# febrianrachmadi/dep-gan-im

Hardware: AMD Instinct MI355X
Metric: 2D slices/sec (G+2D+GP train step), 256x256x1 fp32 (higher is better)
Workload: dtype f32; 1 GPU; DEP-GAN-IM twoCritics canonical train step (critic-Y2 + critic-DEM + G update, WGAN-GP), batch 32 per GPU, 256x256x1; per_gpu_batch=32, global_batch=32, parallelism=dp1

## Files before the change

### dep_gan_im_amd/csrc/igemm_wino.hip

```cpp
#include <stdlib.h>

#include <type_traits>

#include "common.h"
#include "epilogue.h"

namespace {

constexpr int WN_CK = 8;
constexpr int WN_TW = 18;
constexpr int WN_CP = 36;
constexpr int WN_XV = WN_CK / 4;

template <int MT>
struct WnCfg {
  static constexpr int TH = 8 * MT;
  static constexpr int NTILE = 32 * MT;
  static constexpr int PIXT = (TH + 2) * WN_TW;
  static constexpr int XTOT = PIXT * WN_XV;
  static constexpr int NXP = (XTOT + 255) / 256;
  static constexpr int RAW = NXP * 256 * 4;
  static constexpr int VPLANE = NTILE * WN_CK;
  static constexpr int V = 16 * VPLANE;
  static constexpr int ZPLANE = NTILE * WN_CP + 32;
  static constexpr int Z = 8 * ZPLANE;
  static constexpr size_t LDS = sizeof(float) * (size_t)((2 * RAW + V) > Z ? (2 * RAW + V) : Z);
  static constexpr int WGS_PER_CU = (MT == 2) ? 2 : 3;
};

static __device__ __forceinline__ int rslot(int pix, int half) { return (2 * pix + half) ^ (((pix >> 2) & 1) << 1); }

static __device__ __forceinline__ int vslot(int T, int cg, int a) { return ((2 * T + cg) ^ ((T >> 2) & 1) ^ (a << 1)) << 2; }

template <int MT, bool PERS, bool HEAD, int ABL = 0>
static __device__ __forceinline__ void wino_body(const ConvArgs& a) {
  typedef WnCfg<MT> C;
  constexpr int MF = 32, NT = 32;
  constexpr int WN_RAW = C::RAW, WN_VPLANE = C::VPLANE, WN_ZPLANE = C::ZPLANE, WN_XTOT = C::XTOT, NXP = C::NXP;
  typedef f32x16 acc_t;
  extern __shared__ __attribute__((aligned(16))) float smem[];
  float* const raw0 = smem;
  float* const raw1 = smem + WN_RAW;
  float* V = smem + 2 * WN_RAW;

  const int tid = threadIdx.x;
  const int lane = tid & 63, wv = tid >> 6;
  const int r = lane & 31, h = lane >> 5;
  const int tilesX = (a.W + 15) >> 4, tilesY = (a.H + C::TH - 1) / C::TH;
  const unsigned nNTall = (unsigned)a.lgy, nPix = (unsigned)a.lgx;
  const int nCC = a.Cin / WN_CK;

  constexpr int SENT = (int)0x80000000;
  int xvo[NXP], xyx[NXP];
#pragma unroll
  for (int i = 0; i < NXP; ++i) {
    const int q = tid + i * 256;
    const int lq = q ^ (((q >> 3) & 1) << 1);
    const int pix = lq >> 1, part = lq & 1;
    const int ly = pix / WN_TW, lx = pix - ly * WN_TW;
    xvo[i] = (q < WN_XTOT) ? 4 * (ly * (int)a.in.sY + lx * (int)a.in.sX + part * 4) : SENT;
    xyx[i] = (ly << 8) | lx;
  }
  int tA[MT][4], tB[MT][4], tV[MT];
  float tS[MT];
#pragma unroll
  for (int i = 0; i < MT; ++i) {
    const int q = lane + 64 * i;
    const int cg = q & 1, aa = wv, T = q >> 1;
    const int tyi = T >> 3, txi = T & 7;
    const int rA = (aa == 0) ? 0 : (aa == 2 ? 2 : 1), rB = (aa == 3) ? 3 : (aa == 2 ? 1 : 2);
#pragma unroll
    for (int j = 0; j < 4; ++j) {
      tA[i][j] = 4 * rslot((2 * tyi + rA) * WN_TW + 2 * txi + j, cg);
      tB[i][j] = 4 * rslot((2 * tyi + rB) * WN_TW + 2 * txi + j, cg);
    }
    tV[i] = (4 * aa) * WN_VPLANE + vslot(T, cg, aa);
    tS[i] = (aa == 1) ? 1.f : -1.f;
  }
  const int wbase = __builtin_amdgcn_readfirstlane(wv * 256);
  int aoff[MT];
#pragma unroll
  for (int mt = 0; mt < MT; ++mt) aoff[mt] = vslot(32 * mt + r, h, wv);
  const int boff = (4 * wv * 32 + r) * WN_CK + 4 * h;

  unsigned id = blockIdx.x;
  do {
    int t, ntile;
    if ((nPix & 7u) == 0) {
      const unsigned x = id & 7u, sl = id >> 3;
      ntile = (int)(sl % nNTall);
      t = (int)(x * (nPix >> 3) + sl / nNTall);
    } else {
      t = (int)(id % nPix);
      ntile = (int)(id / nPix);
    }
    const int tx0 = (t % tilesX) * 16;
    t /= tilesX;
    const int ty0 = (t % tilesY) * C::TH;
    const int b = t / tilesY;
    const long out_goff = 0;
    const int n0 = ntile * NT;
    const float* inb = a.in.p + (long)b * a.in.sB;
    const bool interior = ty0 >= 1 && ty0 + C::TH + 1 <= a.H && tx0 >= 1 && tx0 + 17 <= a.W;
    const char* halo0 = reinterpret_cast<const char*>(inb + ((long)(ty0 - 1) * a.in.sY + (long)(tx0 - 1) * a.in.sX));
    auto coff = [&](int cc) -> long {
      if (a.cpt > 0) {
        const int run = cc / a.cpt;
        return a.in_run_off[run] + (long)(cc - run * a.cpt) * WN_CK;
      }
      return (long)cc * WN_CK;
    };
    const float* const xorg = a.in.p - ((long)a.in.sY + (long)a.in.sX);
    const unsigned long long xu = (unsigned long long)xorg;
    const unsigned xlo = __builtin_amdgcn_readfirstlane((unsigned)xu), xhi = __builtin_amdgcn_readfirstlane((unsigned)(xu >> 32));
    const __amdgpu_buffer_rsrc_t rx =
        __builtin_amdgcn_make_buffer_rsrc((void*)(((unsigned long long)xhi << 32) | xlo), 0, 0x7FFFFFFF, 0x00020000);
    const int xso0 = 4 * (b * (int)a.in.sB + ty0 * (int)a.in.sY + tx0 * (int)a.in.sX);
    auto stage_dma = [&](int cc, int buf) {
      const int xso = xso0 + 4 * (int)coff(cc);
      float* xs = (buf ? raw1 : raw0) + wbase;
      if (interior) {
#pragma unroll
        for (int i = 0; i < NXP; ++i) {
          const int vo = xvo[i];
          __builtin_amdgcn_raw_ptr_buffer_load_lds(rx, (__attribute__((address_space(3))) void*)(xs + i * 1024), 16, vo,
                                                   xso, 0, 0);
        }
      } else {
#pragma unroll
        for (int i = 0; i < NXP; ++i) {
          const int iy = ty0 + (xyx[i] >> 8) - 1, ix = tx0 + (xyx[i] & 255) - 1;
          const int vo = (iy >= 0 && iy < a.H && ix >= 0 && ix < a.W) ? xvo[i] : SENT;
          __builtin_amdgcn_raw_ptr_buffer_load_lds(rx, (__attribute__((address_space(3))) void*)(xs + i * 1024), 16, vo,
                                                   xso, 0, 0);
        }
      }
    };

    acc_t acc[4][MT];

    const float* wnt = a.w + (size_t)ntile * nCC * (16 * NT * WN_CK) + boff;
    if (!(ABL & 8)) stage_dma(0, 0);
    auto chunk = [&](const int cc, auto first_tag) {
      constexpr bool FIRST = decltype(first_tag)::value;
      f32x4 bq[4];
#pragma unroll
      for (int f = 0; f < 4; ++f)
        bq[f] = *reinterpret_cast<const f32x4*>(wnt + (size_t)cc * (16 * NT * WN_CK) + f * (NT * WN_CK));
      asm volatile("s_waitcnt vmcnt(0)" ::: "memory");
      __syncthreads();
      if (!(ABL & 8) && cc + 1 < nCC) stage_dma(cc + 1, (cc + 1) & 1);
      const float* raw = (cc & 1) ? raw1 : raw0;
#pragma unroll
      for (int i = 0; i < ((ABL & 2) ? 0 : MT); ++i) {
        f32x4 tc[4];
#pragma unroll
        for (int j = 0; j < 4; ++j) {
          const f32x4 x = *reinterpret_cast<const f32x4*>(raw + tA[i][j]);
          const f32x4 y = *reinterpret_cast<const f32x4*>(raw + tB[i][j]);
#pragma unroll
          for (int k = 0; k < 4; ++k) tc[j][k] = fmaf(y[k], tS[i], x[k]);
        }
        f32x4 v0, v1, v2, v3;
#pragma unroll
        for (int k = 0; k < 4; ++k) {
          v0[k] = tc[0][k] - tc[2][k];
          v1[k] = tc[1][k] + tc[2][k];
          v2[k] = tc[2][k] - tc[1][k];
          v3[k] = tc[1][k] - tc[3][k];
        }
        *reinterpret_cast<f32x4*>(V + tV[i]) = v0;
        *reinterpret_cast<f32x4*>(V + tV[i] + WN_VPLANE) = v1;
        *reinterpret_cast<f32x4*>(V + tV[i] + 2 * WN_VPLANE) = v2;
        *reinterpret_cast<f32x4*>(V + tV[i] + 3 * WN_VPLANE) = v3;
      }
      f32x4 av[2][MT];
      auto load_a = [&](int f, f32x4* d) {
#pragma unroll
        for (int mt = 0; mt < MT; ++mt)
          d[mt] = *reinterpret_cast<const f32x4*>(V + (4 * wv + f) * WN_VPLANE + aoff[mt]);
      };
      load_a(0, av[0]);
#pragma unroll
      for (int f = 0; f < 4; ++f) {
        if (f + 1 < 4) load_a(f + 1, av[(f + 1) & 1]);
        __builtin_amdgcn_sched_barrier(0);
#pragma unroll
        for (int j = 0; j < 4; ++j)
#pragma unroll
          for (int mt = 0; mt < MT; ++mt)
            if (!(ABL & 4)) {
              if (FIRST && j == 0) {
                const acc_t zero = {0.f, 0.f, 0.f, 0.f, 0.f, 0.f, 0.f, 0.f, 0.f, 0.f, 0.f, 0.f, 0.f, 0.f, 0.f, 0.f};
                acc[f][mt] = __builtin_amdgcn_mfma_f32_32x32x2f32(bq[f][j], av[f & 1][mt][j], zero, 0, 0, 0);
              } else {
                acc[f][mt] = __builtin_amdgcn_mfma_f32_32x32x2f32(bq[f][j], av[f & 1][mt][j], acc[f][mt], 0, 0, 0);
              }
            } else {
              if (FIRST && j == 0) acc[f][mt] = acc_t{};
              acc[f][mt][j] += bq[f][j] * av[f & 1][mt][j];
            }
        __builtin_amdgcn_sched_barrier(0);
      }
    };
    chunk(0, std::true_type{});
    for (int cc = 1; cc < nCC; ++cc) chunk(cc, std::false_type{});

    if (ABL & 1) {
      float sacc = 0.f;
#pragma unroll
      for (int f = 0; f < 4; ++f)
#pragma unroll
        for (int mt = 0; mt < MT; ++mt)
#pragma unroll
          for (int j = 0; j < 16; ++j) sacc += acc[f][mt][j];
      if (sacc == 12345.678f) a.out.p[tid] = sacc;
      __syncthreads();
      continue;
    }
    auto zstage = [&]() {
      __syncthreads();
      float* zw = smem + (2 * wv) * WN_ZPLANE + r * WN_CP + 4 * h;
#pragma unroll
      for (int mt = 0; mt < MT; ++mt)
#pragma unroll
        for (int g = 0; g < 4; ++g) {
          f32x4 z0, z1;
#pragma unroll
          for (int k = 0; k < 4; ++k) {
            const float m0 = acc[0][mt][4 * g + k], m1 = acc[1][mt][4 * g + k], m2 = acc[2][mt][4 * g + k],
                        m3 = acc[3][mt][4 * g + k];
            z0[k] = (m0 + m1) + m2;
            z1[k] = (m1 - m2) - m3;
          }
          *reinterpret_cast<f32x4*>(zw + mt * (32 * WN_CP) + 8 * g) = z0;
          *reinterpret_cast<f32x4*>(zw + WN_ZPLANE + mt * (32 * WN_CP) + 8 * g) = z1;
        }
      __syncthreads();
    };
#define EPI_PRE_SYNC
#define EPI_STAGE
#define EPI_STAGE_LATE zstage()
#define EPI_NPASS (4 * MT)
#define EPI_OYW (ty0 + 2 * MT * __builtin_amdgcn_readfirstlane(wv))
#define EPI_FULL ((ty0 + C::TH <= a.H) && (tx0 + 16 <= a.W))
#define EPI_FETCH(v, py, px)                                                                                         \
  {                                                                                                                  \
    const float* zb = smem + ((px)&1) * WN_ZPLANE +                                                                  \
                      ((MT * __builtin_amdgcn_readfirstlane(wv) + ((py) >> 1)) * 8 + ((px) >> 1)) * WN_CP + c4;       \
    const f32x4 za = *reinterpret_cast<const f32x4*>(zb + (((py)&1) ? 2 : 0) * WN_ZPLANE);                           \
    const f32x4 zb1 = *reinterpret_cast<const f32x4*>(zb + (((py)&1) ? 4 : 2) * WN_ZPLANE);                          \
    const f32x4 zc = *reinterpret_cast<const f32x4*>(zb + (((py)&1) ? 6 : 4) * WN_ZPLANE);                           \
    _Pragma("unroll") for (int k_ = 0; k_ < 4; ++k_) v[k_] = ((py)&1) ? (za[k_] - zb1[k_]) - zc[k_] : (za[k_] + zb1[k_]) + zc[k_]; \
  }
#define EPI_HEAD HEAD
#include "igemm_epilogue.inc"
#undef EPI_HEAD
#undef EPI_FETCH
#undef EPI_FULL
#undef EPI_OYW
#undef EPI_NPASS
#undef EPI_STAGE_LATE
#undef EPI_STAGE
#undef EPI_PRE_SYNC
    if (PERS) __syncthreads();
  } while (PERS && (id += gridDim.x) < nPix * nNTall);
}

template <int MT, bool PERS>
__global__ __launch_bounds__(256, WnCfg<MT>::WGS_PER_CU) void wino_conv_kernel(const ConvArgs a) {
  wino_body<MT, PERS, false>(a);
}
template <bool PERS>
__global__ __launch_bounds__(256, 2) void wino_conv_head_kernel(const ConvArgs a) {
  wino_body<2, PERS, true>(a);
}
#ifdef DEPGAN_WINO_ABLATIONS
template <int MT, int ABL>
__global__ __launch_bounds__(256, WnCfg<MT>::WGS_PER_CU) void wino_conv_abl_kernel(const ConvArgs a) {
  wino_body<MT, true, false, ABL>(a);
}
#endif

}

bool dg_conv_wino_supported(const ConvPlan& pl, const ConvArgs& a) {
  if (!dg_plan_wino(pl)) return false;
  if (a.Cin != pl.Cin || (a.Cin % WN_CK) || (a.Cout % 32) || a.groups > 1 || a.dbg || ((a.H | a.W) & 1)) return false;
  if (a.cpt > 0 && ((a.Cin % (a.cpt * WN_CK)) != 0 || a.Cin / (a.cpt * WN_CK) > 4)) return false;
  return true;
}

static int wino_mt(const ConvArgs& a) {
  static int forced = -1;
  if (forced < 0) {
    const char* e = getenv("DEPGAN_WINO_MT");
    forced = e ? atoi(e) : 0;
  }
  if (a.ep.head_out) return 2;
  if (forced == 1 || forced == 2) return forced;
  return 1;
}

template <int MT>
static void wino_geometry(ConvArgs& a, long* total, long* G, bool* pers) {
  a.lgx = cdiv(a.W, 16) * cdiv(a.H, WnCfg<MT>::TH) * a.B;
  a.lgy = a.Cout / 32;
  *total = (long)a.lgx * a.lgy;
  const long cap = (long)WnCfg<MT>::WGS_PER_CU * dg_cu_count();
  *pers = *total > cap;
  *G = *pers ? cap : *total;
}

const char* dg_conv_wino_name(const ConvArgs& a_in) {
  ConvArgs a = a_in;
  long total, G;
  bool pers;
  const int mt = wino_mt(a);
  if (mt == 2) wino_geometry<2>(a, &total, &G, &pers); else wino_geometry<1>(a, &total, &G, &pers);
  if (a.ep.head_out) return pers ? "wino_conv_head_kernel<true>" : "wino_conv_head_kernel<false>";
  if (mt == 2) return pers ? "wino_conv_kernel<2,true>" : "wino_conv_kernel<2,false>";
  return pers ? "wino_conv_kernel<1,true>" : "wino_conv_kernel<1,false>";
}

template <int MT>
static int wino_launch(ConvArgs a, hipStream_t st) {
  long total, G;
  bool pers;
  wino_geometry<MT>(a, &total, &G, &pers);
  constexpr size_t LDS = WnCfg<MT>::LDS;
  static DgOncePerDevice once;
  if (once.need()) {
    HIPCHECK(hipFuncSetAttribute(reinterpret_cast<const void*>(&wino_conv_kernel<MT, false>),
                                 hipFuncAttributeMaxDynamicSharedMemorySize, (int)LDS));
    HIPCHECK(hipFuncSetAttribute(reinterpret_cast<const void*>(&wino_conv_kernel<MT, true>),
                                 hipFuncAttributeMaxDynamicSharedMemorySize, (int)LDS));
    if (MT == 2) {
      HIPCHECK(hipFuncSetAttribute(reinterpret_cast<const void*>(&wino_conv_head_kernel<false>),
                                   hipFuncAttributeMaxDynamicSharedMemorySize, (int)LDS));
      HIPCHECK(hipFuncSetAttribute(reinterpret_cast<const void*>(&wino_conv_head_kernel<true>),
                                   hipFuncAttributeMaxDynamicSharedMemorySize, (int)LDS));
    }
  }
#ifdef DEPGAN_WINO_ABLATIONS
  if (const char* e = getenv("DEPGAN_WINO_ABL")) {
    const int abl = atoi(e);
    if (abl && pers && !a.ep.head_out) {
#define WN_ABL_CASE(N)                                                                                              \
  case N:                                                                                                           \
    HIPCHECK(hipFuncSetAttribute(reinterpret_cast<const void*>(&wino_conv_abl_kernel<MT, N>),                       \
                                 hipFuncAttributeMaxDynamicSharedMemorySize, (int)LDS));                            \
    hipLaunchKernelGGL((wino_conv_abl_kernel<MT, N>), dim3((unsigned)G), dim3(256), LDS, st, a);                    \
    break;
// ... 32 lines not shown
```

### dep_gan_im_amd/csrc/op_entries.hip

```cpp
#include "model.h"
#include "train_ops.h"

#include <math.h>
#include <stdlib.h>
#include <stdio.h>
#include <string.h>

int op_pack_jobs(PackJob* jobs, int n, hipStream_t st) {
  const unsigned nb = dg_pack_layout(jobs, n);
  DevTmp jd(st);
  DGCHECK(jd.alloc(n * sizeof(PackJob)));
  hipError_t e = hipMemcpyAsync(jd.p, jobs, n * sizeof(PackJob), hipMemcpyHostToDevice, st);
  if (e != hipSuccess) { dg_set_error("op_pack_jobs: upload failed: %s", hipGetErrorString(e)); return DG_ERR_HIP; }
  return dg_pack_weights_batch(jd.as<PackJob>(), n, nb, st);
}

extern "C" {

static int op_conv_run(ConvArgs a, const float* w_hwio, int Cin, int Cout, int KS, int path, int bwd, hipStream_t st) {
  const int ci = a.Cin, co = a.Cout;
  ConvPlan pl = (path == 3) ? dg_plan_conv_bf16(KS, ci, co)
                : (path == 4 || path == 5) ? dg_plan_conv_split(KS, ci, co, path == 5 ? 3 : 2)
                : (path == 6) ? dg_plan_conv_items(KS, ci, co, 1L << 30) : dg_plan_conv(KS, ci, co);
  if (path == 7) pl = dg_plan_conv_items(KS, ci, co, 1L << 30);
// ... 60 lines not shown
}

int depgan_op_conv2d(const float* in, const float* w_hwio, const float* bias, float* out, int B, int H, int W,
                     int Cin, int Cout, int KS, int relu, int path, void* stream) {
  return op_conv(in, w_hwio, bias, out, B, H, W, Cin, Cout, KS, relu, path, 0, (hipStream_t)stream);
}
int depgan_op_conv2d_bwd_data(const float* dy, const float* w_hwio, float* dx, int B, int H, int W, int Cin,
                              int Cout, int KS, int path, void* stream) {
  return op_conv(dy, w_hwio, nullptr, dx, B, H, W, Cin, Cout, KS, 0, path, 1, (hipStream_t)stream);
}
int depgan_op_conv2d_wgrad(const float* x, const float* dy, float* dw, int B, int H, int W, int Cin, int Cout, int KS,
                           void* stream) {
  hipStream_t st = (hipStream_t)stream;
  const bool big = (Cin % 4 == 0 && Cout % 4 == 0 && Cin >= 8);
  const size_t pf = big ? dg_wgrad_part_floats(KS, B, H, W, Cin, Cout) : dg_wgrad_small_part_floats(KS, B, H, W, Cin, Cout);
  DevTmp part(st);
  DGCHECK(part.alloc(pf * sizeof(float)));
  WgradArgs a = wgrad_args(make_view(const_cast<float*>(x), H, W, Cin), make_view(const_cast<float*>(dy), H, W, Cout),
                           part.as<float>(), B, H, W, Cin, Cout);
  int nch = 0;
  DGCHECK(big ? dg_wgrad(KS, a, &nch, st) : dg_wgrad_small(KS, a, &nch, st));
  return dg_wgrad_reduce(a.part, nch, KS * KS, Cin, Cout, nullptr, dw, nullptr, 0, 0, st);
}
int depgan_op_conv2d_wgrad_bf16(const float* x, const float* dy, float* dw, int B, int H, int W, int Cin, int Cout,
                                int KS, void* stream) {
  hipStream_t st = (hipStream_t)stream;
  if (!dg_wgrad_bf16_supported(KS, Cin, Cout)) { dg_set_error("op_wgrad_bf16: shape not covered"); return DG_ERR_UNSUPPORTED; }
  const size_t pf = dg_wgrad_bf16_part_floats(KS, B, H, W, Cin, Cout);
  DevTmp part(st);
  DGCHECK(part.alloc(pf * sizeof(float)));
  WgradArgs a = wgrad_args(make_view(const_cast<float*>(x), H, W, Cin), make_view(const_cast<float*>(dy), H, W, Cout),
                           part.as<float>(), B, H, W, Cin, Cout);
  int nch = 0;
  DGCHECK(dg_wgrad_bf16(KS, a, &nch, st));
  return dg_wgrad_reduce(a.part, nch, KS * KS, Cin, Cout, nullptr, dw, nullptr, 0, 0, st);
}
int depgan_op_deconv2x2(const float* in, const float* w_hwoi, const float* bias, const float* scale,
                        const float* shift, float* out, int B, int H, int W, int Cin, int Cout, int relu,
                        void* stream) {
  if (!in || !w_hwoi || !out || B < 1 || H < 1 || W < 1) { dg_set_error("op_deconv2x2: bad argument"); return DG_ERR_ARG; }
  DeconvArgs d;
  memset(&d, 0, sizeof(d));
  d.in = in;
  d.w = w_hwoi;
  d.out = make_view(out, 2 * H, 2 * W, Cout);
  d.bias = bias; d.scale = scale; d.shift = shift; d.relu = relu;
  d.H = H; d.W = W; d.Cin = Cin; d.Cout = Cout;
  return dg_deconv_fwd(d, B, (hipStream_t)stream);
}
int depgan_op_deconv2x2_wgrad(const float* in, const float* dout, float* dw_hwoi, float* colsum, int B, int H, int W,
                              int Cin, int Cout, void* stream) {
  if (!in || !dout || !dw_hwoi || B < 1 || H < 1 || W < 1) { dg_set_error("op_deconv2x2_wgrad: bad argument"); return DG_ERR_ARG; }
  hipStream_t st = (hipStream_t)stream;
  DeconvWgradArgs d;
  memset(&d, 0, sizeof(d));
  d.in = in;
  d.dout = make_view(const_cast<float*>(dout), 2 * H, 2 * W, Cout);
  d.H = H; d.W = W; d.Cin = Cin; d.Cout = Cout;
  if (!dg_deconv_wgrad_supported(B, H, W, Cin, Cout, make_view(const_cast<float*>(in), H, W, Cin), d.dout)) {
    dg_set_error("op_deconv2x2_wgrad: shape %dx%dx%d %d->%d not covered by the fused kernel", B, H, W, Cin, Cout);
    return DG_ERR_UNSUPPORTED;
  }
  const size_t pf = dg_deconv_wgrad_part_floats(B, H, W, Cin, Cout);
  DevTmp part(st), col(st);
  DGCHECK(part.alloc(pf * sizeof(float)));
  if (col.alloc((pf / ((size_t)Cin * Cout)) * Cout * sizeof(float)) != DG_OK) {
    dg_set_error("op_deconv2x2_wgrad: out of memory");
    return DG_ERR_HIP;
  }
  d.part = part.as<float>();
  d.colpart = colsum ? col.as<float>() : nullptr;
  int nch = 0;
  DGCHECK(dg_deconv_wgrad(d, B, &nch, st));
  return dg_wgrad_finish_rows(d.part, nch, 4, Cin, Cout, nullptr, dw_hwoi, nullptr, 0, 1, d.colpart, 4 * nch, Cout, nullptr,
                              colsum, nullptr, st);
}
int depgan_op_maxpool(const float* in, float* out, int B, int Ho, int Wo, int C, void* stream) {
  return dg_maxpool(make_view(const_cast<float*>(in), 2 * Ho, 2 * Wo, C), make_view(out, Ho, Wo, C), B, Ho, Wo, C,
                    (hipStream_t)stream);
}

int depgan_eval_accumulate(const float* pred, const float* mask, double* acc, long n, void* stream) {
  if (!pred || !acc || n < 0) { dg_set_error("eval_accumulate: null argument"); return DG_ERR_ARG; }
  return dg_eval_accumulate(pred, mask, acc, (size_t)n, (hipStream_t)stream);
}
int depgan_eval_divide(double* acc, long n, double divisor, void* stream) {
  if (!acc || n < 0) { dg_set_error("eval_divide: null argument"); return DG_ERR_ARG; }
  return dg_eval_divide(acc, (size_t)n, divisor, (hipStream_t)stream);
}
int depgan_eval_counts(const float* x, int nicg, const double* pred, const float* code_real, const float* mask1,
                       const float* wmh1, const float* mask2, const float* wmh2, const float* prob2, long npix,
                       double thr, long long out_host[DEPGAN_EVAL_NCOUNT], void* stream) {
  if (!x || !pred || !out_host || nicg < 1 || npix < 0) { dg_set_error("eval_counts: bad argument"); return DG_ERR_ARG; }
  hipStream_t st = (hipStream_t)stream;
  DevTmp dev(st);
  DGCHECK(dev.alloc(DEPGAN_EVAL_NCOUNT * sizeof(unsigned long long)));
  DGCHECK(dg_eval_counts(x, nicg, pred, code_real, mask1, wmh1, mask2, wmh2, prob2, (size_t)npix, thr,
                         dev.as<unsigned long long>(), st));
  unsigned long long h[DEPGAN_EVAL_NCOUNT];
  if (hipMemcpyAsync(h, dev.p, sizeof(h), hipMemcpyDeviceToHost, st) != hipSuccess ||
      hipStreamSynchronize(st) != hipSuccess) {
    dg_set_error("eval_counts: copy back failed");
    return DG_ERR_HIP;
  }
  for (int k = 0; k < DEPGAN_EVAL_NCOUNT; ++k) out_host[k] = (long long)h[k];
  return DG_OK;
}


static int op_alloc(DevTmp* t, size_t floats, const char* who) {
  if (t->alloc((floats ? floats : 1) * sizeof(float)) != DG_OK) {
    dg_set_error("%s: out of device memory (%zu floats)", who, floats);
    return DG_ERR_HIP;
  }
  return DG_OK;
}
static size_t op_scratch(long scratch_floats, size_t need) { return scratch_floats > 0 ? (size_t)scratch_floats : need; }


int depgan_op_conv2d_fused(const float* in, long isB, long isY, long isX, const float* w_hwio, const float* bias,
                           const float* scale, const float* shift, const float* film_mul, const float* film_add,
                           int film_ld, float* out, long osB, long osY, long osX, float* out_pre, long psB, long psY,
                           long psX, const float* res, long rsB, long rsY, long rsX, const float* mask, long msB,
                           long msY, long msX, float* pool, long qsB, long qsY, long qsX, const float* head_w,
                           const float* head_b, float* head_out, int head_tanh, int head_skip_out, int B, int H, int W,
                           int Cin, int Cout, int KS, int relu, int accumulate, int path, int bwd, void* stream) {
  if (op_view_bad_batched(in, isB, isY, isX) || op_view_bad_batched(out, osB, osY, osX) || !w_hwio || B < 1 || H < 1 || W < 1 || Cin < 1 ||
      Cout < 1 || (KS != 1 && KS != 3 && KS != 5) || (out_pre && op_view_bad_batched(out_pre, psB, psY, psX)) ||
      (res && op_view_bad_batched(res, rsB, rsY, rsX)) || (mask && op_view_bad_batched(mask, msB, msY, msX)) ||
      (pool && op_view_bad_batched(pool, qsB, qsY, qsX))) {
    dg_set_error("op_conv2d_fused: null or non-positive argument");
    return DG_ERR_ARG;
  }
  const int co = bwd ? Cin : Cout;
  if (!scale != !shift || !film_mul != !film_add || (film_mul && film_ld < co)) {
    dg_set_error("op_conv2d_fused: scale / shift and film_mul / film_add come in pairs, film_ld >= output channels");
    return DG_ERR_ARG;
  }
  if ((head_w || head_b || head_out) && !(head_w && head_b && head_out)) { dg_set_error("op_conv2d_fused: null head argument"); return DG_ERR_ARG; }
  if (head_skip_out && !head_out) { dg_set_error("op_conv2d_fused: head_skip_out without a head"); return DG_ERR_ARG; }
  if (path < 1 || path > 10) { dg_set_error("op_conv2d_fused: path must be 1 ... 10"); return DG_ERR_ARG; }
  ConvArgs a = conv_args(op_view(in, isB, isY, isX), op_view(out, osB, osY, osX), B, H, W, bwd ? Cout : Cin, co);
  Epilogue& e = a.ep;
  e.bias = bias; e.scale = scale; e.shift = shift;
  e.film_mul = film_mul; e.film_add = film_add; e.film_ld = film_ld;
  e.out_pre = op_view_or_null(out_pre, psB, psY, psX);
  e.res = op_view_or_null(res, rsB, rsY, rsX);
  e.mask = op_view_or_null(mask, msB, msY, msX);
  e.pool = op_view_or_null(pool, qsB, qsY, qsX);
  e.relu = relu; e.accumulate = accumulate;
  e.head_w = head_w; e.head_b = head_b; e.head_out = head_out;
  e.head_tanh = head_tanh; e.head_skip_out = head_skip_out;
  return op_conv_run(a, w_hwio, Cin, Cout, KS, path, bwd ? 1 : 0, (hipStream_t)stream);
}


int depgan_op_deconv2x2_igemm(int form, const float* in, long isB, long isY, long isX, const float* w_hwoi,
                              const float* bias, const float* scale, const float* shift, float* out, long osB, long osY,
                              long osX, const float* mask, long msB, long msY, long msX, int B, int H, int W, int Cin,
                              int Cout, int relu, int path, void* stream) {
  if (op_view_bad_batched(in, isB, isY, isX) || op_view_bad_batched(out, osB, osY, osX) || !w_hwoi || B < 1 || H < 1 || W < 1 || Cin < 1 ||
      Cout < 1 || (mask && op_view_bad_batched(mask, msB, msY, msX))) {
    dg_set_error("op_deconv2x2_igemm: null or non-positive argument");
    return DG_ERR_ARG;
  }
  if (form < 0 || form > 2 || !scale != !shift || (path != 1 && path != 3 && path != 8)) {
    dg_set_error("op_deconv2x2_igemm: form must be 0, 1 or 2, path 1, 3 or 8, scale and shift come as a pair");
    return DG_ERR_ARG;
  }
  if (form == 0 ? mask != nullptr : (bias || scale || relu)) {
    dg_set_error("op_deconv2x2_igemm: the forward takes bias / scale / shift / relu, the backward-data forms a mask");
    return DG_ERR_ARG;
  }
  if (path == 8) { dg_set_error("op_deconv2x2_igemm: the Winograd kernel has no 1x1 form"); return DG_ERR_UNSUPPORTED; }
  auto plan = [&](int ci, int co) { return path == 3 ? dg_plan_conv_bf16(1, ci, co) : dg_plan_conv(1, ci, co); };
  auto covered = [&](const ConvPlan& p) { return dg_plan_mfma(p) && (path == 3) == dg_plan_bf16(p); };
  hipStream_t st = (hipStream_t)stream;
  ConvArgs a = conv_args(null_view(), null_view(), B, H, W, 0, 0);
  DevTmp wt(st);
  if (form == 0) {
    const ConvPlan pf = plan(Cin, Cout);
    if (!covered(pf)) { dg_set_error("op_deconv2x2_igemm: no MFMA plan for %d -> %d on path %d", Cin, Cout, path); return DG_ERR_UNSUPPORTED; }
    const TView o = op_view(out, osB, osY, osX);
    a.in = op_view(in, isB, isY, isX);
    a.Cin = Cin; a.Cout = Cout;
    a.ep.bias = bias; a.ep.scale = scale; a.ep.shift = shift; a.ep.relu = relu;
    DGCHECK(wt.alloc(4 * pf.packedFloats * sizeof(float)));
    const float* panels[4];
    for (int t = 0; t < 4; ++t) {
      float* dst = wt.as<float>() + (size_t)t * pf.packedFloats;
      DGCHECK(dg_pack_weights(pf, w_hwoi + (size_t)t * Cout * Cin, Cin, Cout, 1, 0, 0, nullptr, dst, st));
      panels[t] = dst;
    }
    deconv_groups(&a, o, panels);
    return dg_conv_igemm(pf, a, st);
  }
  const ConvPlan pb = plan(Cout, Cin);
  if (!covered(pb)) { dg_set_error("op_deconv2x2_igemm: no MFMA plan for %d -> %d on path %d", Cout, Cin, path); return DG_ERR_UNSUPPORTED; }
  const TView d = op_view(in, isB, isY, isX);
  a.out = op_view(out, osB, osY, osX);
  a.Cout = Cin;
  a.ep.mask = op_view_or_null(mask, msB, msY, msX);
  if (form == 1) {
    const ConvPlan pbf = plan(4 * Cout, Cin);
    if (!(pbf.family == pb.family && pbf.planes == pb.planes && (Cout % pb.CK) == 0 && pbf.packedFloats == 4 * pb.packedFloats)) {
      dg_set_error("op_deconv2x2_igemm: the gathered 1x1 form does not cover %d -> %d", Cout, Cin);
      return DG_ERR_UNSUPPORTED;
    }
    DGCHECK(wt.alloc(pbf.packedFloats * sizeof(float)));
    const size_t blk = (size_t)pb.nCC * pb.NT * pb.CK;
    PackJob jobs[4];
    for (int t = 0; t < 4; ++t) {
      float* dst = reinterpret_cast<float*>(wt.as<char>() + t * blk * dg_plan_elem_bytes(pb));
      DGCHECK(dg_pack_job(pb, w_hwoi + (size_t)t * Cout * Cin, Cin, Cout, 1, 1, 0, nullptr, dst, 4 * blk, &jobs[t]));
    }
    DGCHECK(op_pack_jobs(jobs, 4, st));
    deconv_gather_k(&a, d, Cout, pb.CK);
    a.w = wt.as<float>();
    return dg_conv_igemm(pbf, a, st);
  }
  DGCHECK(wt.alloc(4 * pb.packedFloats * sizeof(float)));
  a.Cin = Cout;
  for (int t = 0; t < 4; ++t) {
    float* dst = wt.as<float>() + (size_t)t * pb.packedFloats;
    DGCHECK(dg_pack_weights(pb, w_hwoi + (size_t)t * Cout * Cin, Cin, Cout, 1, 1, 0, nullptr, dst, st));
    a.in = strided2(d, t / 2, t % 2);
    a.w = dst;
    a.ep.accumulate = (t > 0);
    DGCHECK(dg_conv_igemm(pb, a, st));
  }
  return DG_OK;
}

int depgan_op_conv2d_wgrad_ex(const float* x, long xsB, long xsY, long xsX, const float* dy, long dsB, long dsY,
                              long dsX, const float* scale, float* dw, float* raw, int accumulate, int oi,
                              int colB, const float* colscale, float* colout, float* colraw, int B, int H, int W,
                              int Cin, int Cout, int KS, int bf16, void* stream) {
  if (op_view_bad_batched(x, xsB, xsY, xsX) || op_view_bad_batched(dy, dsB, dsY, dsX) || !dw || B < 1 || H < 1 || W < 1 || Cin < 1 || Cout < 1 ||
      (KS != 1 && KS != 3 && KS != 5)) {
    dg_set_error("op_conv2d_wgrad_ex: null or non-positive argument");
    return DG_ERR_ARG;
  }
  const bool cols = colout || colraw;
  if ((bf16 != 0 && bf16 != 1) || (cols ? (colB < 1 || colB > B) : (colB != 0 || colscale != nullptr))) {
    dg_set_error("op_conv2d_wgrad_ex: bf16 must be 0 or 1; column sums need colout or colraw and 1 <= colB <= B");
    return DG_ERR_ARG;
  }
  const bool mfma = Cin % 4 == 0 && Cout % 4 == 0 && Cin >= 8;
  if (bf16 && !(mfma && dg_wgrad_bf16_supported(KS, Cin, Cout))) {
    dg_set_error("op_conv2d_wgrad_ex: the bf16 weight-gradient kernel does not cover %d -> %d", Cin, Cout);
    return DG_ERR_UNSUPPORTED;
  }
  hipStream_t st = (hipStream_t)stream;
  WgradWs ws;
  memset(&ws, 0, sizeof(ws));
  ws.partFloats = bf16 ? dg_wgrad_bf16_part_floats(KS, B, H, W, Cin, Cout)
                  : mfma ? dg_wgrad_part_floats(KS, B, H, W, Cin, Cout) : dg_wgrad_small_part_floats(KS, B, H, W, Cin, Cout);
  ws.scratchFloats = mfma ? ws.partFloats / ((size_t)KS * KS * Cin) : (cols ? dg_colsum_scratch(colB, H, W, Cout) : 0);
  ws.bf16 = bf16 != 0;
  ws.st = st;
  DevTmp part(st), scratch(st);
  DGCHECK(op_alloc(&part, ws.partFloats, "op_conv2d_wgrad_ex"));
  DGCHECK(op_alloc(&scratch, ws.scratchFloats, "op_conv2d_wgrad_ex"));
  ws.part = part.as<float>();
  ws.scratch = scratch.as<float>();
  const ColSum cs = {colB, colscale, colout, colraw};
  return wgrad_run(ws, KS, op_view(x, xsB, xsY, xsX), op_view(dy, dsB, dsY, dsX), B, H, W, Cin, Cout, scale, dw, raw, accumulate,
                   oi, cols ? &cs : nullptr);
}

int depgan_debug_wgrad_plan(int kernel, int KS, int B, int H, int W, int Cin, int Cout, int out[4]) {
  if (!out || B < 1 || H < 1 || W < 1 || Cin < 1 || Cout < 1) {
    dg_set_error("debug_wgrad_plan: null or non-positive argument");
    return DG_ERR_ARG;
  }
  switch (kernel) {
    case 0: return dg_wgrad_plan(KS, B, H, W, Cin, Cout, out);
    case 1: return dg_wgrad_small_plan(KS, B, H, W, Cin, Cout, out);
    case 2: return dg_wgrad_bf16_plan(KS, B, H, W, Cin, Cout, out);
    case 3: return dg_wgrad_bf16s_plan(KS, B, H, W, Cin, Cout, out);
    case 4: return dg_deconv_wgrad_plan(B, H, W, Cin, Cout, out);
  }
  dg_set_error("debug_wgrad_plan: kernel %d is not one of 0..4", kernel);
  return DG_ERR_ARG;
}


int depgan_op_bn_moments(const float* x, long sB, long sY, long sX, int B, int H, int W, int C, float* mean, float* var,
                         long scratch_floats, void* stream) {
  if (!x || !mean || !var || B < 1 || H < 1 || W < 1 || C < 4) { dg_set_error("op_bn_moments: bad argument"); return DG_ERR_ARG; }
  hipStream_t st = (hipStream_t)stream;
  const size_t cap = op_scratch(scratch_floats, dg_col_moments_scratch(B, H, W, C));
  DevTmp scratch(st);
  DGCHECK(op_alloc(&scratch, cap, "op_bn_moments"));
  return dg_col_moments(op_view(x, sB, sY, sX), B, H, W, C, mean, var, scratch.as<float>(), cap, st);
}

int depgan_op_bn_backward(const float* dy, const float* raw, float* draw, long sB, long sY, long sX, int B, int H, int W,
                          int C, const float* gamma, const float* mean, const float* var, float eps, float invN,
                          float dyscale, float* dgamma, float* dbeta, long scratch_floats, void* stream) {
  if (!dy || !raw || !draw || !gamma || !mean || !var || !dgamma || !dbeta || B < 1 || H < 1 || W < 1 || C < 4) {
    dg_set_error("op_bn_backward: bad argument");
    return DG_ERR_ARG;
  }
  hipStream_t st = (hipStream_t)stream;
  const size_t cap = op_scratch(scratch_floats, dg_colsum_pair_scratch(B, H, W, C));
// ... 334 lines not shown
```

### include/depgan.h

```cpp
#ifndef DEPGAN_H
#define DEPGAN_H
#include <stddef.h>
#ifdef __cplusplus
extern "C" {
#endif

typedef struct depgan_ctx depgan_ctx;

#define DEPGAN_ABI_VERSION 3
int depgan_abi_version(void);
size_t depgan_config_size(void);
const char* depgan_source_hash(void);

typedef struct depgan_config {
  int struct_size;
  int batch;
  int height;
  int width;
  int nicg;
  int first_fm;
  float im_thresh;
  float delta;
  float lrD, lrG;
  float beta1, beta2, adam_eps;
// ... 30 lines not shown
float* depgan_arena_ptr(depgan_ctx* ctx, int net, int arena);
int depgan_weights_changed(depgan_ctx* ctx, int net);

int depgan_g_forward(depgan_ctx* ctx, const float* x_dev, const float* z_dev, float* out_dev, int n);
int depgan_d_forward(depgan_ctx* ctx, int net, const float* img_dev, float* out_dev, int n);

int depgan_critic_grads(depgan_ctx* ctx, int net, const float* y2_dev, const float* x_dev, const float* z_dev,
                        const float* ep_dev, float out_host[2]);
int depgan_critic_step(depgan_ctx* ctx, int net, const float* y2_dev, const float* x_dev, const float* z_dev,
                       const float* ep_dev, float out_host[2]);
int depgan_g_eval(depgan_ctx* ctx, const float* x_dev, const float* y2_dev, const float* z_dev, float out_host[6]);
int depgan_g_grads(depgan_ctx* ctx, const float* x_dev, const float* y2_dev, const float* z_dev, float out_host[6]);
#define DEPGAN_MAX_MULTI 32
int depgan_g_eval_multi(depgan_ctx* ctx, const float* x_dev, const float* y2_dev, const float* z_all_dev, int k,
                        float* out_host, float* sums_host);
int depgan_g_step(depgan_ctx* ctx, const float* x_dev, const float* y2_dev, const float* z_dev, float out_host[6]);
int depgan_apply_adam(depgan_ctx* ctx, int net);
long depgan_get_adam_step(depgan_ctx* ctx, int net);
int depgan_set_adam_step(depgan_ctx* ctx, int net, long t);

#define DEPGAN_MAX_CRITIC_STEPS 256
int depgan_gen_iteration(depgan_ctx* ctx, const float* x_y2, const float* y2_y2, const float* z_y2, const float* ep_y2,
                         int n_y2, const float* x_dem, const float* y2_dem, const float* z_dem, const float* ep_dem,
                         int n_dem, long batch_stride, const float* x_gen, const float* y2_gen, const float* z_gen, int k,
                         float* out_host, int* best_host);

int depgan_uresnet_grads(depgan_ctx* ctx, const float* x_dev, const float* z_dev, const float* labels_dev, int n,
                         unsigned drop_seed, float* loss_host);
int depgan_uresnet_step(depgan_ctx* ctx, const float* x_dev, const float* z_dev, const float* labels_dev, int n,
                        unsigned drop_seed, float* loss_host);
int depgan_uresnet_eval(depgan_ctx* ctx, const float* x_dev, const float* z_dev, const float* labels_dev, int n,
                        float* loss_host);

int depgan_last_sums(depgan_ctx* ctx, float out_host[8]);

int depgan_profile_enable(depgan_ctx* ctx, int on);
int depgan_profile_read(depgan_ctx* ctx, int klass, double* total_ms, long* launches, double* flops);
int depgan_profile_read_bytes(depgan_ctx* ctx, int klass, double* bytes);
int depgan_profile_reset(depgan_ctx* ctx);
int depgan_profile_dump(depgan_ctx* ctx, const char* path);

#define DEPGAN_EVAL_NCOUNT 20
int depgan_eval_accumulate(const float* pred_dev, const float* mask_dev, double* acc_dev, long n, void* stream);
int depgan_eval_divide(double* acc_dev, long n, double divisor, void* stream);
int depgan_eval_counts(const float* x_dev, int nicg, const double* pred_dev, const float* code_real_dev,
                       const float* mask1_dev, const float* wmh1_dev, const float* mask2_dev, const float* wmh2_dev,
                       const float* prob2_dev, long npix, double thr, long long out_host[DEPGAN_EVAL_NCOUNT],
                       void* stream);

size_t depgan_data_prep_scratch_floats(int X, int Y, int Z);
int depgan_data_prep_subject(const float* p1_dev, const float* f1_dev, const float* icv1_dev, const float* sl1_dev,
                             const float* p2_dev, const float* icv2_dev, const float* sl2_dev, int X, int Y, int Z,
                             int nicg, float* x_out_dev, float* y2_out_dev, float* scratch_dev, void* stream);

#define DEPGAN_MAX_CLASSES 127
#define DEPGAN_EVAL_LABEL_NCOUNT 18
size_t depgan_data_zscore_scratch_floats(int X, int Y, int Z);
int depgan_data_prep_zscore(const float* f1_dev, const float* icv1_dev, const float* sl1_dev, int X, int Y, int Z,
                            float* flair_out_dev, float* stats_out_dev, float* scratch_dev, void* stream);
int depgan_data_mask_slices(const float* vol_dev, const float* m_a_dev, const float* sl_dev, int X, int Y, int Z,
                            float* out_dev, void* stream);
int depgan_labels_to_onehot(const float* coded_dev, long npix, int C, float* onehot_out_dev, void* stream);
int depgan_eval_accumulate_channels(const float* pred_dev, const float* mask_dev, double* acc_dev, long npix, int C,
                                    void* stream);
int depgan_eval_label_counts(const double* pred_dev, int C, const float* code_real_dev, const float* mask1_dev,
                             const float* wmh1_dev, const float* mask2_dev, const float* wmh2_dev, long npix,
                             signed char* labels_out_dev, long long out_host[DEPGAN_EVAL_LABEL_NCOUNT], void* stream);

int depgan_debug_capture(depgan_ctx* ctx, int on);
int depgan_debug_tensor(depgan_ctx* ctx, const char* name, float* host_dst, long cap_floats, int shape[4]);

int depgan_g_forward_bf16s(depgan_ctx* ctx, const float* x_dev, const float* z_dev, float* out_dev, int n);
int depgan_debug_tensor_bf16s(depgan_ctx* ctx, const char* name, float* host_dst, long cap_floats, int shape[4]);

int depgan_set_fwd_only_storage(depgan_ctx* ctx, int storage);
int depgan_get_fwd_only_storage(depgan_ctx* ctx);

int depgan_set_g_update_storage(depgan_ctx* ctx, int storage);
int depgan_get_g_update_storage(depgan_ctx* ctx);

int depgan_set_critic16_pipe(depgan_ctx* ctx, int pipe);
int depgan_get_critic16_pipe(depgan_ctx* ctx);
int depgan_debug_film_decision_bf16s(depgan_ctx* ctx, const char* layer, unsigned char* host_dst, long cap_bytes,
                                     int shape[4]);

int depgan_op_conv2d_film_train_bf16s(const void* in, long isB, long isY, long isX, const float* w_hwio, const float* bias,
                                      const float* scale, const float* shift, const float* film_mul, const float* film_add,
                                      int film_ld, const void* res, long rsB, long rsY, long rsX, void* out, long osB,
                                      long osY, long osX, void* u_out, unsigned char* dec_bits, int B, int H, int W, int Cin,
                                      int Cout, int relu, void* hip_stream);
int depgan_op_conv2d_wgrad_bf16s(const void* x, long xsB, long xsY, long xsX, const float* dy, long dsB, long dsY, long dsX,
                                 float* dw, float* colsum, int B, int H, int W, int Cin, int Cout, int KS, int oi,
                                 void* hip_stream);
int depgan_op_conv2d_bwd_data_bf16s(const float* dy, long dsB, long dsY, long dsX, const float* w, const float* res,
                                    long rsB, long rsY, long rsX, const void* mask, long msB, long msY, long msX, float* dx,
                                    long osB, long osY, long osX, int B, int H, int W, int Cin, int Cout, int deconv,
                                    void* hip_stream);
int depgan_op_unpool_mask_bf16s(const float* dpool, long dsB, long dsY, long dsX, const void* a, long asB, long asY, long asX,
                                const float* skip, long ssB, long ssY, long ssX, float* out, long osB, long osY, long osX,
                                int B, int Ho, int Wo, int C, void* hip_stream);
int depgan_op_film_bwd_bf16s(const float* dr, const void* u, const unsigned char* dec_bits, const float* fmul, int film_ld,
                             float* du, float* dmul, float* dadd, int B, long HW, int C, void* hip_stream);
int depgan_op_head_bwd_bf16s(int backward, const void* a, long ld, const float* w, const float* dpre, float* out, long P,
                             int C, void* hip_stream);

int depgan_op_conv2d_bf16s(const void* in, long isB, long isY, long isX, const float* w_hwio, const float* bias,
                           const float* scale, const float* shift, const float* film_mul, const float* film_add,
                           int film_ld, const void* res, long rsB, long rsY, long rsX, void* out, long osB, long osY,
                           long osX, void* pool, int B, int H, int W, int Cin, int Cout, int KS, int relu,
                           void* hip_stream);
int depgan_op_conv2d_head_bf16s(const void* in, long isB, long isY, long isX, const float* w_hwio, const float* bias,
                                const float* scale, const float* shift, const float* film_mul, const float* film_add,
                                int film_ld, const void* res, long rsB, long rsY, long rsX, void* out, long osB,
                                long osY, long osX, void* pool, int B, int H, int W, int Cin, int Cout, int KS, int relu,
                                const float* head_w, const float* head_b, float* head_out, int tanh_act, int skip_out,
                                void* hip_stream);
int depgan_op_deconv2x2_bf16s(const void* in, long isB, long isY, long isX, const float* w_hwoi, const float* bias,
                              const float* scale, const float* shift, void* out, long osB, long osY, long osX, int B,
                              int H, int W, int Cin, int Cout, int relu, void* hip_stream);
int depgan_op_edge_conv_bf16s(const float* in, const float* w_hwio, const float* bias, const float* scale,
                              const float* shift, void* out, long osB, long osY, long osX, int B, int H, int W, int Cin,
                              int Cout, int relu, void* hip_stream);
int depgan_op_head_bf16s(const void* a, const float* w, const float* b, float* out, long P, int C, int tanh_act,
                         void* hip_stream);
int depgan_op_head_softmax_bf16s(const void* a, long ld, const float* w, const float* b, float* probs,
                                 float* logits_or_null, long P, int C, void* hip_stream);

int depgan_op_conv2d(const float* in, const float* w_hwio, const float* bias, float* out, int B, int H, int W,
                     int Cin, int Cout, int KS, int relu, int path, void* hip_stream);
int depgan_op_conv2d_bwd_data(const float* dy, const float* w_hwio, float* dx, int B, int H, int W, int Cin,
                              int Cout, int KS, int path, void* hip_stream);
int depgan_op_conv2d_wgrad(const float* x, const float* dy, float* dw_hwio, int B, int H, int W, int Cin, int Cout,
                           int KS, void* hip_stream);
int depgan_op_conv2d_wgrad_bf16(const float* x, const float* dy, float* dw_hwio, int B, int H, int W, int Cin,
                                int Cout, int KS, void* hip_stream);

int depgan_op_conv2d_stamps(const float* in, const float* w_hwio, float* out, int B, int H, int W, int Cin, int Cout,
                            int KS, unsigned long long* stamps, int reps, void* hip_stream);
int depgan_op_maxpool(const float* in, float* out, int B, int Ho, int Wo, int C, void* hip_stream);
int depgan_op_deconv2x2(const float* in, const float* w_hwoi, const float* bias, const float* scale,
                        const float* shift, float* out, int B, int H, int W, int Cin, int Cout, int relu,
                        void* hip_stream);

int depgan_op_deconv2x2_wgrad(const float* in, const float* dout, float* dw_hwoi, float* colsum, int B, int H, int W,
                              int Cin, int Cout, void* hip_stream);

int depgan_op_conv2d_fused(const float* in, long isB, long isY, long isX, const float* w_hwio, const float* bias,
                           const float* scale, const float* shift, const float* film_mul, const float* film_add,
                           int film_ld, float* out, long osB, long osY, long osX, float* out_pre, long psB, long psY,
                           long psX, const float* res, long rsB, long rsY, long rsX, const float* mask, long msB,
                           long msY, long msX, float* pool, long qsB, long qsY, long qsX, const float* head_w,
                           const float* head_b, float* head_out, int head_tanh, int head_skip_out, int B, int H, int W,
                           int Cin, int Cout, int KS, int relu, int accumulate, int path, int bwd, void* hip_stream);
int depgan_op_deconv2x2_igemm(int form, const float* in, long isB, long isY, long isX, const float* w_hwoi,
                              const float* bias, const float* scale, const float* shift, float* out, long osB, long osY,
                              long osX, const float* mask, long msB, long msY, long msX, int B, int H, int W, int Cin,
                              int Cout, int relu, int path, void* hip_stream);
int depgan_op_conv2d_wgrad_ex(const float* x, long xsB, long xsY, long xsX, const float* dy, long dsB, long dsY,
                              long dsX, const float* scale, float* dw, float* raw, int accumulate, int oi, int colB,
                              const float* colscale, float* colout, float* colraw, int B, int H, int W, int Cin,
                              int Cout, int KS, int bf16, void* hip_stream);
int depgan_debug_wgrad_plan(int kernel, int KS, int B, int H, int W, int Cin, int Cout, int out[4]);

int depgan_op_bn_moments(const float* x, long sB, long sY, long sX, int B, int H, int W, int C, float* mean, float* var,
                         long scratch_floats, void* hip_stream);
int depgan_op_bn_backward(const float* dy, const float* raw, float* draw, long sB, long sY, long sX, int B, int H, int W,
                          int C, const float* gamma, const float* mean, const float* var, float eps, float invN,
                          float dyscale, float* dgamma, float* dbeta, long scratch_floats, void* hip_stream);
int depgan_op_affine_act(const float* in, float* out, float* out_pre, const float* res, long sB, long sY, long sX,
                         const float* s, const float* t, const float* film_mul, const float* film_add, int film_ld,
                         int relu, int B, int H, int W, int C, unsigned drop_seed, float drop_rate, void* hip_stream);
int depgan_op_softmax_ce4(const float* logits, const float* onehot, float* probs, float* dz, float* loss_sum, long P,
                          void* hip_stream);
int depgan_op_bn_rows_fwd(const float* x, float* y, int R, int C, int ld, const float* gamma, const float* beta,
                          float eps, float momentum, float corr, float* moving_mean, float* moving_var, float* mean,
                          float* rstd, int relu, void* hip_stream);
int depgan_op_bn_rows_bwd(const float* dy, const float* x, const float* relu_out, float* dx, int R, int C, int ld,
                          const float* gamma, const float* mean, const float* rstd, float* dgamma, float* dbeta,
                          void* hip_stream);
int depgan_op_small_gemm(int form, const float* A, const float* Bm, const float* bias, float* Cm, int M, int K, int N,
                         void* hip_stream);

int depgan_op_unpool_mask(const float* dpool, long dsB, long dsY, long dsX, const float* a, long asB, long asY, long asX,
                          const float* skip, long ssB, long ssY, long ssX, float* out, long osB, long osY, long osX,
                          int B, int Ho, int Wo, int C, void* hip_stream);
int depgan_op_gather_pool(const float* u, long usB, long usY, long usX, const float* a, long asB, long asY, long asX,
                          float* out, long osB, long osY, long osX, int B, int Ho, int Wo, int C, void* hip_stream);
int depgan_op_head(int backward, const float* a, const float* w, const float* b, const float* dpre, float* out, long P,
                   int C, int tanh_act, void* hip_stream);
int depgan_op_critic_tail_fwd(const float* a, const float* w9, const float* b9, const float* wd, const float* bd,
                              float* t9, float* out, int N, int HW, int C, void* hip_stream);
int depgan_op_critic_tail_bwd(const float* a, const float* w9, const float* wd, const float* coefs, int per, float* dz,
                              int N, int HW, int C, void* hip_stream);
int depgan_op_critic_tail_wgrad(const float* src, const float* w9, const float* b9, const float* wd, const float* coefs,
                                int per, int add_bias_terms, int accumulate, float* dw9, float* db9, float* dwd,
                                float* dbd, int N, int HW, int C, long scratch_floats, void* hip_stream);
int depgan_op_colsum(const float* v, long sB, long sY, long sX, int B, int H, int W, int C, const float* scale,
                     float* out, float* raw, int accumulate, const float* rowmul, long scratch_floats, void* hip_stream);
int depgan_op_sum(const float* in, long n, float* out, long scratch_floats, void* hip_stream);
int depgan_op_critic_inputs(const float* y2, const float* x, int nicg, const float* attr, const float* ep, float* out,
                            int B, long HW, int which, void* hip_stream);
int depgan_op_gp_u0(const float* g0, float* u0, float* norms, float* gp_out, float delta, int B, long HW,
                    long scratch_floats, void* hip_stream);
int depgan_op_critic_stats(const float* d_out, const float* norms, float* out, int B, void* hip_stream);
int depgan_op_gloss_sums(const float* x, int nicg, const float* y2, const float* attr, float thr, float* sums, long P,
                         long scratch_floats, void* hip_stream);
int depgan_op_g_dpre(const float* x, int nicg, const float* y2, const float* attr, const float* g1, const float* g2,
                     float* dpre, int B, long P, void* hip_stream);
int depgan_op_film_bwd(const float* dr, const float* u, const float* fmul, const float* fadd, int film_ld, float* du,
                       float* dmul, float* dadd, int B, long HW, int C, long scratch_floats, void* hip_stream);
int depgan_op_bn_prepare_batch(void* const* ptrs, const int* C, int njobs, float eps, void* hip_stream);
int depgan_op_bn_gamma_grad_batch(void* const* ptrs, const int* dims, int njobs, void* hip_stream);
int depgan_op_noise_fwd(const float* trunk, const float* Wh, const float* hvec, const int* ncol, const float* z,
                        float* acts, int B, void* hip_stream);
int depgan_op_noise_bwd(const float* trunk, const float* Wh, const float* hvec, const int* ncol, const float* z,
                        float* acts, const float* dheads, float* gtrunk, float* dWh, float* ghvec, int B,
                        long scratch_floats, void* hip_stream);
int depgan_op_best_noise(const float* stats, int k, const float* z_all, long zfloats, int* best, float* z_out,
                         void* hip_stream);
int depgan_op_round_bf16_masked(const float* src, const unsigned char* mask, float* dst, long n, void* hip_stream);

#ifdef __cplusplus
}
#endif
#endif
```

Before: 654.6 slices/s.

## Feed Winograd input transform directly into MFMA registers, dropping V LDS stage

The Winograd conv kernel no longer writes transformed input tiles to an LDS V buffer and reads them back. Each lane now computes exactly the transformed values its own MFMA operands need, keeps them in registers, and uses packed f32x2 FMAs. The raw LDS swizzle is changed to match the new access pattern. This removes the LDS round trip and shrinks the LDS footprint, at the cost of extra registers. The diff also adds a new gathered Winograd conv entry point that references fields (cpt, in_run_off) not shown being defined.

```diff
diff --git a/dep_gan_im_amd/csrc/igemm_wino.hip b/dep_gan_im_amd/csrc/igemm_wino.hip
--- a/dep_gan_im_amd/csrc/igemm_wino.hip
+++ b/dep_gan_im_amd/csrc/igemm_wino.hip
@@ -20,28 +20,25 @@
   static constexpr int XTOT = PIXT * WN_XV;
   static constexpr int NXP = (XTOT + 255) / 256;
   static constexpr int RAW = NXP * 256 * 4;
-  static constexpr int VPLANE = NTILE * WN_CK;
-  static constexpr int V = 16 * VPLANE;
+  static_assert(XTOT % 4 == 0 && WN_TW % 2 == 0, "rslot permutes inside aligned groups of four slots: halo and padding stay apart");
   static constexpr int ZPLANE = NTILE * WN_CP + 32;
   static constexpr int Z = 8 * ZPLANE;
-  static constexpr size_t LDS = sizeof(float) * (size_t)((2 * RAW + V) > Z ? (2 * RAW + V) : Z);
+  static constexpr size_t LDS = sizeof(float) * (size_t)((2 * RAW) > Z ? (2 * RAW) : Z);
   static constexpr int WGS_PER_CU = (MT == 2) ? 2 : 3;
 };
 
-static __device__ __forceinline__ int rslot(int pix, int half) { return (2 * pix + half) ^ (((pix >> 2) & 1) << 1); }
-
-static __device__ __forceinline__ int vslot(int T, int cg, int a) { return ((2 * T + cg) ^ ((T >> 2) & 1) ^ (a << 1)) << 2; }
+static __device__ __forceinline__ int rslot(int pix, int half) { return (2 * pix + half) ^ (((pix % WN_TW) >> 2) & 3); }
+static __device__ __forceinline__ int rslot_inv(int q) { return q ^ ((((q >> 1) % WN_TW) >> 2) & 3); }
 
 template <int MT, bool PERS, bool HEAD, int ABL = 0>
 static __device__ __forceinline__ void wino_body(const ConvArgs& a) {
   typedef WnCfg<MT> C;
   constexpr int MF = 32, NT = 32;
-  constexpr int WN_RAW = C::RAW, WN_VPLANE = C::VPLANE, WN_ZPLANE = C::ZPLANE, WN_XTOT = C::XTOT, NXP = C::NXP;
+  constexpr int WN_RAW = C::RAW, WN_ZPLANE = C::ZPLANE, WN_XTOT = C::XTOT, NXP = C::NXP;
   typedef f32x16 acc_t;
   extern __shared__ __attribute__((aligned(16))) float smem[];
   float* const raw0 = smem;
   float* const raw1 = smem + WN_RAW;
-  float* V = smem + 2 * WN_RAW;
 
   const int tid = threadIdx.x;
   const int lane = tid & 63, wv = tid >> 6;
@@ -55,18 +52,17 @@
 #pragma unroll
   for (int i = 0; i < NXP; ++i) {
     const int q = tid + i * 256;
-    const int lq = q ^ (((q >> 3) & 1) << 1);
+    const int lq = rslot_inv(q);
     const int pix = lq >> 1, part = lq & 1;
     const int ly = pix / WN_TW, lx = pix - ly * WN_TW;
     xvo[i] = (q < WN_XTOT) ? 4 * (ly * (int)a.in.sY + lx * (int)a.in.sX + part * 4) : SENT;
     xyx[i] = (ly << 8) | lx;
   }
-  int tA[MT][4], tB[MT][4], tV[MT];
+  int tA[MT][4], tB[MT][4];
   float tS[MT];
 #pragma unroll
   for (int i = 0; i < MT; ++i) {
-    const int q = lane + 64 * i;
-    const int cg = q & 1, aa = wv, T = q >> 1;
+    const int cg = h, aa = wv, T = 32 * i + r;
     const int tyi = T >> 3, txi = T & 7;
     const int rA = (aa == 0) ? 0 : (aa == 2 ? 2 : 1), rB = (aa == 3) ? 3 : (aa == 2 ? 1 : 2);
 #pragma unroll
@@ -74,13 +70,9 @@
       tA[i][j] = 4 * rslot((2 * tyi + rA) * WN_TW + 2 * txi + j, cg);
       tB[i][j] = 4 * rslot((2 * tyi + rB) * WN_TW + 2 * txi + j, cg);
     }
-    tV[i] = (4 * aa) * WN_VPLANE + vslot(T, cg, aa);
     tS[i] = (aa == 1) ? 1.f : -1.f;
   }
   const int wbase = __builtin_amdgcn_readfirstlane(wv * 256);
-  int aoff[MT];
-#pragma unroll
-  for (int mt = 0; mt < MT; ++mt) aoff[mt] = vslot(32 * mt + r, h, wv);
   const int boff = (4 * wv * 32 + r) * WN_CK + 4 * h;
 
   unsigned id = blockIdx.x;
@@ -151,39 +143,40 @@
       __syncthreads();
       if (!(ABL & 8) && cc + 1 < nCC) stage_dma(cc + 1, (cc + 1) & 1);
       const float* raw = (cc & 1) ? raw1 : raw0;
+      f32x2 vr[MT][4][2];
+      if (ABL & 2) {
+#pragma unroll
+        for (int i = 0; i < MT; ++i)
+#pragma unroll
+          for (int bb = 0; bb < 4; ++bb) vr[i][bb][0] = vr[i][bb][1] = f32x2{0.f, 0.f};
+      }
 #pragma unroll
       for (int i = 0; i < ((ABL & 2) ? 0 : MT); ++i) {
-        f32x4 tc[4];
+        const f32x2 s2 = {tS[i], tS[i]};
+        f32x2 tc[4][2];
+        f32x4 xs[4], ys[4];
 #pragma unroll
         for (int j = 0; j < 4; ++j) {
-          const f32x4 x = *reinterpret_cast<const f32x4*>(raw + tA[i][j]);
-          const f32x4 y = *reinterpret_cast<const f32x4*>(raw + tB[i][j]);
-#pragma unroll
-          for (int k = 0; k < 4; ++k) tc[j][k] = fmaf(y[k], tS[i], x[k]);
-        }
-        f32x4 v0, v1, v2, v3;
-#pragma unroll
-        for (int k = 0; k < 4; ++k) {
-          v0[k] = tc[0][k] - tc[2][k];
-          v1[k] = tc[1][k] + tc[2][k];
-          v2[k] = tc[2][k] - tc[1][k];
-          v3[k] = tc[1][k] - tc[3][k];
-        }
-        *reinterpret_cast<f32x4*>(V + tV[i]) = v0;
-        *reinterpret_cast<f32x4*>(V + tV[i] + WN_VPLANE) = v1;
-        *reinterpret_cast<f32x4*>(V + tV[i] + 2 * WN_VPLANE) = v2;
-        *reinterpret_cast<f32x4*>(V + tV[i] + 3 * WN_VPLANE) = v3;
-      }
-      f32x4 av[2][MT];
-      auto load_a = [&](int f, f32x4* d) {
-#pragma unroll
-        for (int mt = 0; mt < MT; ++mt)
-          d[mt] = *reinterpret_cast<const f32x4*>(V + (4 * wv + f) * WN_VPLANE + aoff[mt]);
-      };
-      load_a(0, av[0]);
+          xs[j] = *reinterpret_cast<const f32x4*>(raw + tA[i][j]);
+          ys[j] = *reinterpret_cast<const f32x4*>(raw + tB[i][j]);
+        }
+        __builtin_amdgcn_sched_barrier(0);
+#pragma unroll
+        for (int j = 0; j < 4; ++j) {
+          const f32x4 x = xs[j], y = ys[j];
+          tc[j][0] = __builtin_elementwise_fma(f32x2{y[0], y[1]}, s2, f32x2{x[0], x[1]});
+          tc[j][1] = __builtin_elementwise_fma(f32x2{y[2], y[3]}, s2, f32x2{x[2], x[3]});
+        }
+#pragma unroll
+        for (int p = 0; p < 2; ++p) {
+          vr[i][0][p] = tc[0][p] - tc[2][p];
+          vr[i][1][p] = tc[1][p] + tc[2][p];
+          vr[i][2][p] = tc[2][p] - tc[1][p];
+          vr[i][3][p] = tc[1][p] - tc[3][p];
+        }
+      }
 #pragma unroll
       for (int f = 0; f < 4; ++f) {
-        if (f + 1 < 4) load_a(f + 1, av[(f + 1) & 1]);
         __builtin_amdgcn_sched_barrier(0);
 #pragma unroll
         for (int j = 0; j < 4; ++j)
@@ -192,13 +185,13 @@
             if (!(ABL & 4)) {
               if (FIRST && j == 0) {
                 const acc_t zero = {0.f, 0.f, 0.f, 0.f, 0.f, 0.f, 0.f, 0.f, 0.f, 0.f, 0.f, 0.f, 0.f, 0.f, 0.f, 0.f};
-                acc[f][mt] = __builtin_amdgcn_mfma_f32_32x32x2f32(bq[f][j], av[f & 1][mt][j], zero, 0, 0, 0);
+                acc[f][mt] = __builtin_amdgcn_mfma_f32_32x32x2f32(bq[f][j], vr[mt][f][j >> 1][j & 1], zero, 0, 0, 0);
               } else {
-                acc[f][mt] = __builtin_amdgcn_mfma_f32_32x32x2f32(bq[f][j], av[f & 1][mt][j], acc[f][mt], 0, 0, 0);
+                acc[f][mt] = __builtin_amdgcn_mfma_f32_32x32x2f32(bq[f][j], vr[mt][f][j >> 1][j & 1], acc[f][mt], 0, 0, 0);
               }
             } else {
               if (FIRST && j == 0) acc[f][mt] = acc_t{};
-              acc[f][mt][j] += bq[f][j] * av[f & 1][mt][j];
+              acc[f][mt][j] += bq[f][j] * vr[mt][f][j >> 1][j & 1];
             }
         __builtin_amdgcn_sched_barrier(0);
       }
diff --git a/dep_gan_im_amd/csrc/op_entries.hip b/dep_gan_im_amd/csrc/op_entries.hip
--- a/dep_gan_im_amd/csrc/op_entries.hip
+++ b/dep_gan_im_amd/csrc/op_entries.hip
@@ -236,6 +236,26 @@
   e.head_w = head_w; e.head_b = head_b; e.head_out = head_out;
   e.head_tanh = head_tanh; e.head_skip_out = head_skip_out;
   return op_conv_run(a, w_hwio, Cin, Cout, KS, path, bwd ? 1 : 0, (hipStream_t)stream);
+}
+
+
+int depgan_op_conv3x3_wino_gathered(const float* in, long isB, long isY, long isX, const long* run_off, int runs,
+                                    const float* w_hwio, const float* bias, float* out, long osB, long osY, long osX,
+                                    int B, int H, int W, int Cin, int Cout, void* stream) {
+  if (op_view_bad_batched(in, isB, isY, isX) || op_view_bad_batched(out, osB, osY, osX) || !w_hwio || !run_off || B < 1 || H < 1 ||
+      W < 1 || Cin < 1 || Cout < 1 || runs < 1 || runs > 4) {
+    dg_set_error("op_conv3x3_wino_gathered: null or non-positive argument, or not 1 ... 4 runs");
+    return DG_ERR_ARG;
+  }
+  if (Cin % (runs * 8)) {
+    dg_set_error("op_conv3x3_wino_gathered: %d channels are not %d runs of whole 8-channel chunks", Cin, runs);
+    return DG_ERR_UNSUPPORTED;
+  }
+  ConvArgs a = conv_args(op_view(in, isB, isY, isX), op_view(out, osB, osY, osX), B, H, W, Cin, Cout);
+  a.ep.bias = bias;
+  a.cpt = Cin / (runs * 8);
+  for (int t = 0; t < runs; ++t) a.in_run_off[t] = run_off[t];
+  return op_conv_run(a, w_hwio, Cin, Cout, 3, 8, 0, (hipStream_t)stream);
 }
 
 
diff --git a/include/depgan.h b/include/depgan.h
--- a/include/depgan.h
+++ b/include/depgan.h
@@ -206,6 +206,9 @@
                            long msY, long msX, float* pool, long qsB, long qsY, long qsX, const float* head_w,
                            const float* head_b, float* head_out, int head_tanh, int head_skip_out, int B, int H, int W,
                            int Cin, int Cout, int KS, int relu, int accumulate, int path, int bwd, void* hip_stream);
+int depgan_op_conv3x3_wino_gathered(const float* in, long isB, long isY, long isX, const long* run_off, int runs,
+                                    const float* w_hwio, const float* bias, float* out, long osB, long osY, long osX,
+                                    int B, int H, int W, int Cin, int Cout, void* hip_stream);
 int depgan_op_deconv2x2_igemm(int form, const float* in, long isB, long isY, long isX, const float* w_hwoi,
                               const float* bias, const float* scale, const float* shift, float* out, long osB, long osY,
                               long osX, const float* mask, long msB, long msY, long msX, int B, int H, int W, int Cin,
```

Measured after the change: 665.6 slices/s (median of 6 runs). 1.7% higher.
